# JussiM01/MARL-nav

Hardware: AMD Instinct MI355X
Metric: env-steps/sec (whole node) at 3 agents; 1/2/4/8-GPU scaling + %HBM roofline (higher is better)
Workload: dtype f32

## Files before the change

### marl-nav_amd/csrc/device_math.h

```cpp
#pragma once

__host__ __device__ inline int obs_dim(int A, int O) { return 2 + 2 * O + 2 * (A - 1); }

__device__ __forceinline__ float clamp_t(float x, float lo, float hi)
{
    x = x < lo ? lo : x;
    return x > hi ? hi : x;
}

constexpr bool kNtRows = true;
constexpr bool kNtOther = false;
typedef float v4f_t __attribute__((ext_vector_type(4)));
typedef float v2f_t __attribute__((ext_vector_type(2)));

template <class T>
__device__ __forceinline__ __attribute__((address_space(1))) T *gptr(T *p)
{
    return (__attribute__((address_space(1))) T *)p;
}

template <bool NT = kNtOther, class T>
__device__ __forceinline__ void out_st(T *p, T v)
{
    if constexpr (NT)
// ... 661 lines not shown
#pragma unroll
                for (int l = 0; l < 8; ++l) acc[k][l] += f(x[(4 * r + k) * 8 + l]);
#pragma unroll
        for (int v = 4 * M; v < V; ++v)
#pragma unroll
            for (int l = 0; l < 8; ++l) acc[0][l] += f(x[v * 8 + l]);
#pragma unroll
        for (int k = 1; k < 4; ++k)
#pragma unroll
            for (int l = 0; l < 8; ++l) acc[0][l] += acc[k][l];
        float fin = 0.0f;
#pragma unroll
        for (int i = 8 * V; i < N; ++i) fin += f(x[i]);
#pragma unroll
        for (int l = 0; l < 8; ++l) fin += acc[0][l];
        return fin;
    } else {
        float a0 = 0.0f, a1 = 0.0f, a2 = 0.0f, a3 = 0.0f;
        constexpr int M = N / 4;
#pragma unroll
        for (int r = 0; r < M; ++r) {
            a0 += f(x[4 * r]);
            a1 += f(x[4 * r + 1]);
            a2 += f(x[4 * r + 2]);
            a3 += f(x[4 * r + 3]);
        }
#pragma unroll
        for (int i = 4 * M; i < N; ++i) a0 += f(x[i]);
        a0 += a1;
        a0 += a2;
        a0 += a3;
        return a0;
    }
}

template <bool FAST, bool REFC = false>
__device__ __forceinline__ float bond_term(float d, const MarlnavParams &pr, bool &ok)
{
    if constexpr (FAST) {
        if constexpr (REFC) {
            const float sd = d - pr.ideal_dist;
            return recip_fast(1.0f + sd * sd, ok);
        } else {
            const DivC d_sharp = make_divc(pr.bond_sharpness, ok);
            const float sd = div_c(d - pr.ideal_dist, d_sharp, ok);
            return recip_fast(1.0f + sd * sd, ok);
        }
    } else {
        const float sd = (d - pr.ideal_dist) / pr.bond_sharpness;
        return 1.0f / (1.0f + sd * sd);
    }
}

template <int A, bool FAST, bool REFC>
__device__ __forceinline__ RowOut row_reward(float ta, float td, bool risk_any, bool col_any,
                                             float band, float bond, const MarlnavParams &pr,
                                             bool &ok)
{
    const float head = fabsf(ta) < pr.max_angle_diff ? 1.0f : 0.0f;
    const float bandc = band < pr.max_at_prop_d ? band : pr.max_at_prop_d;
    float dsc, soft;
    if (FAST && (pr.flags & kTermsFastFlag)) {
        const DivC d_init = make_divc(pr.init_dist, ok);
        soft = -1.0f * div_c(td, d_init, ok);
        if constexpr (REFC) {
            dsc = bandc * 0.5f;
        } else {
            const DivC d_mapd = make_divc(pr.max_at_prop_d, ok);
            dsc = div_c(bandc, d_mapd, ok);
        }
    } else {
        dsc = bandc / pr.max_at_prop_d;
        soft = -1.0f * (td / pr.init_dist);
    }
    const float bondm = bond / (float)(A - 1);
    const float risk = risk_any ? 1.0f : 0.0f;
    float rm = pr.target_factor * 0.0f + pr.heading_factor * head;
    float rh = pr.target_factor * 1.0f + pr.heading_factor * head;
    rm = rm + pr.distance_factor * dsc;
    rh = rh + pr.distance_factor * dsc;
    rm = rm + pr.soft_factor * soft;
    rh = rh + pr.soft_factor * soft;
    rm = rm + pr.bond_factor * bondm;
    rh = rh + pr.bond_factor * bondm;
    rm = rm - pr.risk_factor * risk;
    rh = rh - pr.risk_factor * risk;
    return RowOut{rm, rh, (col_any ? 1u : 0u) | ((td < pr.target_radius) ? 2u : 0u)};
}

template <int A, int O, bool TERMS, bool FAST, bool REFC = false>
__device__ __forceinline__ RowOut observe_row_own(const float *__restrict__ sts,
                                                  const float *__restrict__ obe,
                                                  const float *__restrict__ tge, int a,
                                                  float ox, float oy, float dx, float dy,
                                                  float *row, const MarlnavParams &pr, bool &ok)
{
    const float cap = pr.cap_distance;
    if constexpr (FAST) {
        constexpr int NP = 1 + O + (A - 1);
        float px[NP], py[NP], pd[NP], pg[NP];
        px[0] = tge[0];
        py[0] = tge[1];
#pragma unroll
        for (int j = 0; j < O; ++j) {
            px[1 + j] = obe[2 * j];
            py[1 + j] = obe[2 * j + 1];
        }
#pragma unroll
        for (int j = 0; j < A - 1; ++j) {
            const int m = j + (j >= a ? 1 : 0);
            px[1 + O + j] = sts[5 * m];
            py[1 + O + j] = sts[5 * m + 1];
        }
        pairs_fast<NP>(ox, oy, dx, dy, px, py, cap, pd, pg);
        row[0] = pg[0];
        row[1] = pd[0];
        bool ob_risk = false, ob_col = false, ag_risk = false, ag_col = false;
        float band = 0.0f;
#pragma unroll
        for (int j = 0; j < O; ++j) {
            row[2 + j] = pg[1 + j];
            row[2 + O + j] = pd[1 + j];
            if (TERMS) {
                ob_risk |= pd[1 + j] < pr.ob_risk_dist;
                ob_col |= pd[1 + j] < pr.ob_coll_dist;
            }
        }
#pragma unroll
        for (int j = 0; j < A - 1; ++j) {
            const float d = pd[1 + O + j];
            row[2 + 2 * O + j] = pg[1 + O + j];
            row[2 + 2 * O + (A - 1) + j] = d;
            if (TERMS) {
                ag_risk |= d < pr.ag_risk_dist;
                ag_col |= d < pr.ag_coll_dist;
                band += (pr.agents_min_d < d && d < pr.agents_max_d) ? 1.0f : 0.0f;
            }
        }
        RowOut out{0.0f, 0.0f, 0u};
        if (TERMS) {
            const float *agd = row + 2 + 2 * O + (A - 1);
            float bond;
            if (pr.flags & kTermsFastFlag)
                bond = torch_row_sum_r<A - 1>(agd, [&](float d) { return bond_term<true, REFC>(d, pr, ok); });
            else
                bond = torch_row_sum_r<A - 1>(agd, [&](float d) { return bond_term<false>(d, pr, ok); });
            out = row_reward<A, FAST, REFC>(pg[0], pd[0], ob_risk || ag_risk, ob_col || ag_col, band,
                                            bond, pr, ok);
        }
        return out;
    }
    const float td = pair_dist<false>(ox, oy, tge[0], tge[1], ok);
    const float ta = pair_angle<false>(ox, oy, tge[0], tge[1], dx, dy, td, cap, ok);
    row[0] = ta;
    row[1] = td;
    bool ob_risk = false, ob_col = false;
#pragma unroll
    for (int j = 0; j < O; ++j) {
        const float px = obe[2 * j], py = obe[2 * j + 1];
        const float d = pair_dist<false>(ox, oy, px, py, ok);
        row[2 + j] = pair_angle<false>(ox, oy, px, py, dx, dy, d, cap, ok);
        row[2 + O + j] = d;
        if (TERMS) {
            ob_risk |= d < pr.ob_risk_dist;
            ob_col |= d < pr.ob_coll_dist;
        }
    }
    bool ag_risk = false, ag_col = false;
    float band = 0.0f;
#pragma unroll
    for (int j = 0; j < A - 1; ++j) {
        const int m = j + (j >= a ? 1 : 0);
        const float px = sts[5 * m], py = sts[5 * m + 1];
        const float d = pair_dist<false>(ox, oy, px, py, ok);
        row[2 + 2 * O + j] = pair_angle<false>(ox, oy, px, py, dx, dy, d, cap, ok);
        row[2 + 2 * O + (A - 1) + j] = d;
        if (TERMS) {
            ag_risk |= d < pr.ag_risk_dist;
            ag_col |= d < pr.ag_coll_dist;
            band += (pr.agents_min_d < d && d < pr.agents_max_d) ? 1.0f : 0.0f;
        }
    }
    RowOut out{0.0f, 0.0f, 0u};
    if (TERMS) {
        const float *agd = row + 2 + 2 * O + (A - 1);
        const float bond = torch_row_sum_r<A - 1>(agd, [&](float d) { return bond_term<false>(d, pr, ok); });
        out = row_reward<A, false, REFC>(ta, td, ob_risk || ag_risk, ob_col || ag_col, band, bond,
                                         pr, ok);
    }
    return out;
}

template <int A, int O, bool TERMS, bool FAST>
__device__ __forceinline__ RowOut observe_row_regs(const float *__restrict__ sts,
                                                   const float *__restrict__ obe,
                                                   const float *__restrict__ tge, int a,
                                                   float *row, const MarlnavParams &pr,
                                                   bool &ok)
{
    return observe_row_own<A, O, TERMS, FAST>(sts, obe, tge, a, sts[5 * a], sts[5 * a + 1],
                                              sts[5 * a + 2], sts[5 * a + 3], row, pr, ok);
// ... 81 lines not shown
```

### marl-nav_amd/csrc/kernel_args.h

```cpp
#pragma once

typedef __attribute__((address_space(3))) void LdsVoid;

struct KArgs {
    StepArgs a;
    MarlnavParams p;
};
typedef __attribute__((address_space(4))) const KArgs KArgsK;

template <int OFF>
__device__ __forceinline__ KArgsK *kargs_late()
{
    const char *p = (const char *)__builtin_amdgcn_kernarg_segment_ptr() + OFF;
    KArgsK *k = (KArgsK *)p;
    asm volatile("" : "+s"(k));
    return k;
}

constexpr int kHotKargsOff = 7 * 8;

template <class T>
__device__ __forceinline__ T in_sgpr(T p)
{
    asm volatile("" : "+s"(p));
// ... 23 lines not shown
    q.formation = K->a.b.formation;
    return q;
}

__device__ __forceinline__ MarlnavParams load_params(KArgsK *K)
{
    MarlnavParams p;
#define MARLNAV_CP(f) p.f = K->p.f
    MARLNAV_CP(min_speed); MARLNAV_CP(max_speed); MARLNAV_CP(min_accel); MARLNAV_CP(max_accel);
    MARLNAV_CP(trunc_after); MARLNAV_CP(risk_factor); MARLNAV_CP(distance_factor);
    MARLNAV_CP(heading_factor); MARLNAV_CP(target_factor); MARLNAV_CP(soft_factor);
    MARLNAV_CP(bond_factor); MARLNAV_CP(ob_risk_dist); MARLNAV_CP(ag_risk_dist);
    MARLNAV_CP(ob_coll_dist); MARLNAV_CP(ag_coll_dist); MARLNAV_CP(agents_min_d);
    MARLNAV_CP(agents_max_d); MARLNAV_CP(max_at_prop_d); MARLNAV_CP(max_angle_diff);
    MARLNAV_CP(target_radius); MARLNAV_CP(cap_distance); MARLNAV_CP(bond_sharpness);
    MARLNAV_CP(ideal_dist); MARLNAV_CP(init_dist); MARLNAV_CP(obs_range_x);
    MARLNAV_CP(obs_mean_x); MARLNAV_CP(obs_range_y); MARLNAV_CP(obs_mean_y);
    MARLNAV_CP(ags_dist); MARLNAV_CP(noise_std); MARLNAV_CP(angle_range);
    MARLNAV_CP(flags); MARLNAV_CP(seed);
    MARLNAV_CP(act_scale[0]); MARLNAV_CP(act_scale[1]);
    MARLNAV_CP(act_mean[0]); MARLNAV_CP(act_mean[1]);
#undef MARLNAV_CP
    p.reserved = 0;
    return p;
}

template <int NB, int AUX = 0>
__device__ __forceinline__ void glds_span(const void *src, float *dst, unsigned lane)
{
    constexpr int N16 = NB / 16, R4 = (NB % 16) / 4;
#pragma unroll
    for (int k = 0; k * 64 < N16; ++k) {
        const char *s = in_sgpr(reinterpret_cast<const char *>(src) + k * 1024);
        if ((k + 1) * 64 <= N16 || (int)lane < N16 - k * 64)
            __builtin_amdgcn_global_load_lds(s + lane * 16u, (LdsVoid *)(dst + k * 256), 16, 0,
                                             AUX);
    }
    if constexpr (R4 > 0) {
        const char *s = in_sgpr(reinterpret_cast<const char *>(src) + N16 * 16);
        if ((int)lane < R4)
            __builtin_amdgcn_global_load_lds(s + lane * 4u, (LdsVoid *)(dst + N16 * 4), 4, 0,
                                             AUX);
    }
}

typedef float f32x2 __attribute__((ext_vector_type(2)));
__device__ __forceinline__ f32x2 global_load_x2_raw(const float *p)
{
    f32x2 v;
    asm volatile("global_load_dwordx2 %0, %1, off" : "=v"(v) : "v"(p) : "memory");
    return v;
}

__device__ __forceinline__ f32x2 vm_landed(f32x2 v)
{
    asm volatile("" : "+v"(v)::"memory");
    return v;
}

__device__ __forceinline__ void wait_vmcnt(int n)
{
    switch (n) {
    case 0: asm volatile("s_waitcnt vmcnt(0)" ::: "memory"); break;
    case 1: asm volatile("s_waitcnt vmcnt(1)" ::: "memory"); break;
    case 2: asm volatile("s_waitcnt vmcnt(2)" ::: "memory"); break;
    case 3: asm volatile("s_waitcnt vmcnt(3)" ::: "memory"); break;
    case 4: asm volatile("s_waitcnt vmcnt(4)" ::: "memory"); break;
    case 5: asm volatile("s_waitcnt vmcnt(5)" ::: "memory"); break;
    case 6: asm volatile("s_waitcnt vmcnt(6)" ::: "memory"); break;
    case 7: asm volatile("s_waitcnt vmcnt(7)" ::: "memory"); break;
    default: asm volatile("s_waitcnt vmcnt(0)" ::: "memory"); break;
    }
}

template <class T>
__device__ __forceinline__ void copy_span(const T *__restrict__ src, T *__restrict__ dst, int n,
                                          int lane)
{
#pragma clang loop vectorize(disable) unroll(disable)
    for (int i = lane; i < n; i += 64) dst[i] = src[i];
}

__host__ __device__ constexpr int tile_envs(int A) { return (64 / A) >= 4 ? (64 / A) & ~3 : 64 / A; }
```

### marl-nav_amd/csrc/kernel_block.h

```cpp
#pragma once

template <int A, int O>
struct BlockPlan {
    static constexpr int E = 64, R = E * A, D = 2 + 2 * O + 2 * (A - 1);
    static constexpr int NT = 64 * A;
    static constexpr int ST = 0;
    static constexpr int ACTW = (ST + R * 5 + 3) & ~3;
    static constexpr int OB = (ACTW + 2 * R + 3) & ~3;
    static constexpr int TG = (OB + E * O * 2 + 3) & ~3;
    static constexpr int SN = (TG + E * 2 + 3) & ~3;
    static constexpr int TM = (SN + E + 3) & ~3;
    static constexpr int FORM = (TM + E / 4 + 3) & ~3;
    static constexpr int RED = (FORM + 5 * A + 2 + 3) & ~3;
    static constexpr int OBS = RED + 4 * R;
    static constexpr int LIST = (OBS + R * D + 3) & ~3;
    static constexpr int FLG = LIST + E;
    static constexpr int FRESH = (FLG + 1 + A + 3) & ~3;
    static constexpr int FLOATS = FRESH + 2 * O * E;
    static_assert(A >= 2 && A <= 16, "one wave per agent");
};

template <int NB, int AUX = 0>
__device__ __forceinline__ void block_glds(int k, int A, int w, const void *src, float *dst,
                                           unsigned lane)
{
    if (k % A == w) glds_span<NB, AUX>(src, dst, lane);
}

__host__ __device__ constexpr int glds_count(int NB)
{
    return (NB / 16 + 63) / 64 + ((NB % 16) / 4 > 0 ? 1 : 0);
}

template <int A, int O>
struct BlockSpans {
    using BP = BlockPlan<A, O>;
    static constexpr int N = 6;
    static constexpr int K[N] = {0, 1, 4, 2, 5, 7};
    static constexpr int NB[N] = {BP::R * 20, BP::E * O * 8, BP::E * 8, BP::E * 4, BP::E,
                                  (5 * A + 2) * 4};
    static constexpr int after_actions(int w, bool formation)
    {
        int n = 0;
        for (int i = 0; i < N; ++i)
            if (K[i] % A == w && (i != N - 1 || formation)) n += glds_count(NB[i]);
        return n;
    }
};

template <int A, int O, bool OBS_ONLY, int W>
__device__ __forceinline__ void block_stage_wave(const StepPtrs &b, int64_t e0, float *lds,
                                                 unsigned lane, bool formation)
{
    using BP = BlockPlan<A, O>;
    using BS = BlockSpans<A, O>;
    if constexpr (BS::K[0] % A == W)
        glds_span<BS::NB[0]>(b.states + e0 * (A * 5), lds + BP::ST, lane);
    if constexpr (BS::K[1] % A == W)
        glds_span<BS::NB[1]>(b.obstacles + e0 * (O * 2), lds + BP::OB, lane);
    if constexpr (BS::K[2] % A == W) glds_span<BS::NB[2]>(b.target + e0 * 2, lds + BP::TG, lane);
    if constexpr (!OBS_ONLY) {
        if constexpr (BS::K[3] % A == W) glds_span<BS::NB[3]>(b.step_num + e0, lds + BP::SN, lane);
        if constexpr (BS::K[4] % A == W) glds_span<BS::NB[4]>(b.terminates + e0, lds + BP::TM, lane);
        if constexpr (BS::K[5] % A == W)
            if (formation) glds_span<BS::NB[5]>(b.formation, lds + BP::FORM, lane);
    }
}

template <int A, int O, bool OBS_ONLY, int... W>
__device__ __forceinline__ void block_stage_waves(std::integer_sequence<int, W...>, int w,
                                                  const StepPtrs &b, int64_t e0, float *lds,
                                                  unsigned lane, bool formation)
{
    ((w == W ? block_stage_wave<A, O, OBS_ONLY, W>(b, e0, lds, lane, formation) : (void)0), ...);
}

template <int A, int O>
constexpr bool kBlockWaveStage = O < 8;

template <class T>
__device__ __forceinline__ void block_copy(const T *__restrict__ src, T *__restrict__ dst, int n,
                                           int tid, int nt)
{
#pragma clang loop vectorize(disable) unroll(disable)
    for (int i = tid; i < n; i += nt) dst[i] = src[i];
}

__device__ __forceinline__ void block_store(float *__restrict__ dst, const float *__restrict__ src,
                                            int n, int tid, int nt, bool wt)
{
    const int n4 = n >> 2;
    if (wt) {
        const OutBuf ob = out_buf(dst, (uint32_t)n * 4u);
        for (int i = tid; i < n4; i += nt)
            wt_st4(ob, 16u * i, reinterpret_cast<const float4 *>(src)[i]);
        for (int i = (n4 << 2) + tid; i < n; i += nt) wt_st(ob, 4u * i, src[i]);
        return;
    }
    for (int i = tid; i < n4; i += nt)
        out_st4<kNtRows>(dst + 4 * i, reinterpret_cast<const float4 *>(src)[i]);
    for (int i = (n4 << 2) + tid; i < n; i += nt) out_st<kNtRows>(dst + i, src[i]);
}

template <int N1, int N2, int NT>
__device__ __forceinline__ void block_store2(float *__restrict__ d1, const float *__restrict__ s1,
                                             float *__restrict__ d2, const float *__restrict__ s2,
                                             int tid, bool wt)
{
    static_assert(N1 % 4 == 0 && N2 % 4 == 0, "whole 16-byte pieces");
    constexpr int Q1 = N1 / 4, Q2 = N2 / 4, K1 = (Q1 + NT - 1) / NT, K2 = (Q2 + NT - 1) / NT;
    float4 v1[K1], v2[K2];
#pragma unroll
    for (int k = 0; k < K1; ++k)
        if ((k + 1) * NT <= Q1 || tid + k * NT < Q1)
            v1[k] = reinterpret_cast<const float4 *>(s1)[tid + k * NT];
#pragma unroll
    for (int k = 0; k < K2; ++k)
        if ((k + 1) * NT <= Q2 || tid + k * NT < Q2)
            v2[k] = reinterpret_cast<const float4 *>(s2)[tid + k * NT];
    if (wt) {
        const OutBuf o1 = out_buf(d1, N1 * 4), o2 = out_buf(d2, N2 * 4);
#pragma unroll
        for (int k = 0; k < K1; ++k)
            if ((k + 1) * NT <= Q1 || tid + k * NT < Q1) wt_st4(o1, 16u * (tid + k * NT), v1[k]);
#pragma unroll
        for (int k = 0; k < K2; ++k)
            if ((k + 1) * NT <= Q2 || tid + k * NT < Q2) wt_st4(o2, 16u * (tid + k * NT), v2[k]);
        return;
    }
#pragma unroll
    for (int k = 0; k < K1; ++k)
        if ((k + 1) * NT <= Q1 || tid + k * NT < Q1) out_st4<kNtRows>(d1 + 4 * (tid + k * NT), v1[k]);
#pragma unroll
    for (int k = 0; k < K2; ++k)
        if ((k + 1) * NT <= Q2 || tid + k * NT < Q2) out_st4<kNtRows>(d2 + 4 * (tid + k * NT), v2[k]);
}

struct EnvEnd {
    unsigned any_col, all_in;
    float step_num;
    bool truncated, term_old, terminated, fin;
};

template <int A, class F>
__device__ __forceinline__ EnvEnd env_end(F flag, float step_num_old, uint8_t terminates_old,
                                          float trunc_after)
{
    EnvEnd e;
    e.any_col = 0u;
    e.all_in = 1u;
#pragma unroll
    for (int i = 0; i < A; ++i) {
        const unsigned f = flag(i);
        e.any_col |= f & 1u;
        e.all_in &= (f >> 1) & 1u;
    }
    e.step_num = step_num_old + 1.0f;
    e.truncated = e.step_num > trunc_after;
    e.term_old = terminates_old != 0;
    e.terminated = e.any_col != 0u || e.term_old;
    e.fin = e.truncated || e.terminated;
    return e;
}

template <int A, int O, bool HELP>
constexpr bool kBlockEarlyOut = O >= 8 || !HELP;

struct BlockDynamic {
    static constexpr int all_full = -1, write_through = -1, native_overlap = -1,
                         has_formation = -1, no_norm = -1, no_action_scale = -1,
                         default_bond = -1, has_counters = -1;
    static constexpr bool ptrs_early = false;
};

template <bool WT>
struct BlockFixed {
    static constexpr int all_full = 1, write_through = WT, native_overlap = 1, has_formation = 1,
                         no_norm = 1, no_action_scale = 1, default_bond = 1, has_counters = 1;
    static constexpr bool ptrs_early = true;
};


template <int A, int O, bool OBS_ONLY, bool NOISY, bool HELP = false, class FX = BlockDynamic>
__global__ void __launch_bounds__(64 * (A + HELP))
    block_kernel(float *h_states, const float *h_actions, const float *h_obstacles,
                 const float *h_target, const float *h_step_num, const uint8_t *h_terminates,
                 int64_t h_P, KArgs k)
{
    using BP = BlockPlan<A, O>;
    constexpr int E = BP::E, R = BP::R, D = BP::D, NT = BP::NT;
    static_assert(!HELP || (!OBS_ONLY && !NOISY), "the draw wave serves the native re-init step");
    static_assert(FX::native_overlap <= 0 || (!OBS_ONLY && !NOISY), "native_overlap: the native step");
    (void)k;
    extern __shared__ __attribute__((aligned(16))) float lds[];
#if MARLNAV_STAMPS
    unsigned long long t_entry;
    asm volatile("s_memrealtime %0\n\ts_waitcnt lgkmcnt(0)" : "=s"(t_entry));
#endif
    if (MARLNAV_AB & 4096) return;
    const int tid = (int)threadIdx.x;
    const unsigned lane = threadIdx.x & 63;
    const int w = __builtin_amdgcn_readfirstlane(threadIdx.x >> 6);
    const bool hw = HELP && w == A;
    KArgsK *K = kargs_late<kHotKargsOff>();
    const int64_t P = h_P;
    StepPtrs b = load_ptrs(K);
    b.states = h_states;
    b.actions = h_actions;
    b.obstacles = const_cast<float *>(h_obstacles);
    b.target = const_cast<float *>(h_target);
    b.step_num = const_cast<float *>(h_step_num);
    b.terminates = const_cast<uint8_t *>(h_terminates);
    using BS = BlockSpans<A, O>;
    auto block = [&]() __attribute__((always_inline)) {
    const int64_t blk = blockIdx.x;
    const int64_t gw = blk * (A + HELP) + w;
    STAMP(0);
    STAMP_ISSUED_DECL;
    float *st = lds + BP::ST;
    const int64_t e0 = blk * E;
    const int ne = FX::all_full > 0 ? E : (int)((P - e0) < E ? (P - e0) : E);
    const bool full = FX::all_full < 0 ? ne == E : FX::all_full > 0;
    const auto has_form = [&] {
        return FX::has_formation < 0 ? b.formation != nullptr : FX::has_formation > 0;
    };

    constexpr bool WS = kBlockWaveStage<A, O>;
    float *actw = lds + BP::ACTW + 2 * E * (hw ? 0 : w);
    f32x2 act_own = {0.0f, 0.0f};
    if (!OBS_ONLY && full && !hw) {
        const float *pa = h_actions + ((e0 + lane) * A + w) * 2;
        if constexpr (WS) {
            act_own = global_load_x2_raw(pa);
        } else {
            __builtin_amdgcn_global_load_lds(pa, (LdsVoid *)actw, 4, 0, 0);
            __builtin_amdgcn_global_load_lds(pa + 1, (LdsVoid *)(actw + E), 4, 0, 0);
        }
    }
    static_assert(BS::NB[0] == R * 20 && BS::NB[1] == E * O * 8 && BS::NB[2] == E * 8 &&
                      BS::NB[3] == E * 4 && BS::NB[4] == E && BS::NB[5] == (5 * A + 2) * 4,
                  "span table and LDS plan agree");
    if (WS && full) {
        block_stage_waves<A, O, OBS_ONLY>(std::make_integer_sequence<int, A>{}, w, b, e0, lds, lane,
                                          has_form());
    } else if (full) {
        block_glds<BS::NB[0]>(BS::K[0], A, w, b.states + e0 * (A * 5), st, lane);
        block_glds<BS::NB[1]>(BS::K[1], A, w, b.obstacles + e0 * (O * 2), lds + BP::OB, lane);
        block_glds<BS::NB[2]>(BS::K[2], A, w, b.target + e0 * 2, lds + BP::TG, lane);
        if (!OBS_ONLY) {
            block_glds<BS::NB[3]>(BS::K[3], A, w, b.step_num + e0, lds + BP::SN, lane);
            block_glds<BS::NB[4]>(BS::K[4], A, w, b.terminates + e0, lds + BP::TM, lane);
            if (has_form())
                block_glds<BS::NB[5]>(BS::K[5], A, w, b.formation, lds + BP::FORM, lane);
        }
    } else if (!hw) {
        const int nr = ne * A;
        block_copy(b.states + e0 * (A * 5), st, nr * 5, tid, NT);
        if (!OBS_ONLY && (int)lane < ne) {
            const float *pa = h_actions + ((e0 + lane) * A + w) * 2;
            actw[lane] = pa[0];
            actw[E + lane] = pa[1];
        }
        block_copy(b.obstacles + e0 * (O * 2), lds + BP::OB, ne * O * 2, tid, NT);
        block_copy(b.target + e0 * 2, lds + BP::TG, ne * 2, tid, NT);
        if (!OBS_ONLY) {
            block_copy(b.step_num + e0, lds + BP::SN, ne, tid, NT);
            block_copy(b.terminates + e0, reinterpret_cast<uint8_t *>(lds + BP::TM), ne, tid, NT);
            if (has_form()) block_copy(b.formation, lds + BP::FORM, 5 * A + 2, tid, NT);
        }
    }
    STAMP_ISSUED();
    const MarlnavParams pr = load_params(K);
    const bool wt =
        FX::write_through < 0 ? (pr.flags & kWriteThroughFlag) != 0 : FX::write_through > 0;
    const bool overlap = FX::native_overlap < 0 ? !OBS_ONLY && !NOISY && !K->a.b.fresh_states
                                                : FX::native_overlap > 0;
    constexpr bool kPre = E * O <= NT;
    if constexpr (HELP) {
        if (hw && overlap && (int)lane < ne) {
            KArgsK *kl = kargs_late<kHotKargsOff>();
            const uint64_t sidx = kl->a.step_idx, g = (uint64_t)(kl->a.env_offset + e0) + lane;
            float *pre = lds + BP::FRESH;
            float v[O][2];
#pragma unroll
            for (int j = 0; j < O; ++j)
                native_obst_draw(pr.seed, sidx, g, j, pr.obs_range_x, pr.obs_mean_x, pr.obs_range_y,
                                 pr.obs_mean_y, v[j]);
#pragma unroll
            for (int j = 0; j < O; ++j) {
                pre[(2 * j) * E + lane] = v[j][0];
                pre[(2 * j + 1) * E + lane] = v[j][1];
            }
        }
    } else if (kPre && overlap) {
        KArgsK *kl = kargs_late<kHotKargsOff>();
        const uint64_t sidx = kl->a.step_idx, g0 = (uint64_t)(kl->a.env_offset + e0);
        float *pre = lds + BP::FRESH;
#pragma unroll
        for (int k2 = 0; k2 * NT < E * O; ++k2) {
            const int i = tid + k2 * NT;
            const int l = i % E, j = __builtin_amdgcn_readfirstlane(i / E);
            if (((k2 + 1) * NT <= E * O || i < E * O) && l < ne) {
                float v[2];
                native_obst_draw(pr.seed, sidx, g0 + l, j, pr.obs_range_x, pr.obs_mean_x,
                                 pr.obs_range_y, pr.obs_mean_y, v);
                pre[(2 * j) * E + l] = v[0];
                pre[(2 * j + 1) * E + l] = v[1];
            }
        }
    }
    float sn = 0.0f, c = 1.0f, a1 = 0.0f;
    if (!OBS_ONLY && !hw) {
        if (full) {
            int n = 0;
#pragma unroll
            for (int ww = 0; ww < A; ++ww)
                if (w == ww) n = has_form() ? BS::after_actions(ww, true) : BS::after_actions(ww, false);
            wait_vmcnt(n);
        }
        float a0;
        if (WS && full) {
            act_own = vm_landed(act_own);
            a0 = act_own.x;
            a1 = act_own.y;
        } else {
            a0 = actw[lane];
            a1 = actw[E + lane];
        }
        STAMPS_S(0);
        if (FX::no_action_scale < 0 ? (pr.flags & MARLNAV_SCALE_ACTIONS) != 0
                                    : FX::no_action_scale == 0) {
            KArgsK *kl = kargs_late<kHotKargsOff>();
            a0 = kl->p.act_scale[0] * a0 + kl->p.act_mean[0];
            a1 = kl->p.act_scale[1] * a1 + kl->p.act_mean[1];
        }
        sincos_k(clamp_t(a0, -kPiF, kPiF), &sn, &c);
#if MARLNAV_STAMPS && MARLNAV_SUBSTAMPS
        asm volatile("" ::"v"(sn), "v"(c));
#endif
        STAMPS_S(1);
    }
    const int l = (int)lane;
    const int r = l * A + (hw ? 0 : w);
    const bool row_on = l < ne && !hw;
    const int nrow = ne * A;
    int *bad_word = reinterpret_cast<int *>(lds + BP::FLG) + 1;
    if (tid == 0) *bad_word = 0;
    asm volatile("s_waitcnt vmcnt(0)" ::: "memory");
    STAMPS_S(2);
    __syncthreads();
    STAMP(1);
    if (MARLNAV_AB & 8192) {
        asm volatile("" ::"v"(sn), "v"(c), "v"(a1));
        return;
    }

    CoordRange crange;
    if (full && !hw) {
        constexpr int NC = E * O * 2 + E * 2;
        static_assert(BP::TG == BP::OB + E * O * 2, "adjacent obstacle/target spans");
#pragma unroll
        for (int k2 = 0; k2 * NT < NC; ++k2) {
            const int i = tid + k2 * NT;
            if ((k2 + 1) * NT <= NC || i < NC) crange.add(lds[BP::OB + i]);
        }
    }

    float ox, oy, dx, dy;
    {
        const float *s = st + 5 * r;
        ox = s[0];
        oy = s[1];
        dx = s[2];
        dy = s[3];
    }
    if (!OBS_ONLY) {
        const float ndx = c * dx + (-sn) * dy;
        const float ndy = sn * dx + c * dy;
        float *s = st + 5 * r;
        const float v = clamp_t(s[4] + clamp_t(a1, pr.min_accel, pr.max_accel), pr.min_speed,
                                pr.max_speed);
        ox = ox + ndx * v;
        oy = oy + ndy * v;
        dx = ndx;
        dy = ndy;
        if (row_on) {
            s[0] = ox;
            s[1] = oy;
            s[2] = dx;
            s[3] = dy;
            s[4] = v;
        }
    }
    if (full && !hw) {
        crange.add(ox);
        crange.add(oy);
        const bool bad = __ballot(!crange.ok()) != 0ull;
        if (lane == 0 && bad) *bad_word = 1;
    }
    __syncthreads();
    STAMP(2);
    const bool fast = full && *bad_word == 0;

    float4 *red = reinterpret_cast<float4 *>(lds + BP::RED);
    float *obs_rows = lds + BP::OBS;
    if (row_on) {
        float rowv[D];
        RowOut ro;
        bool unused = true;
        if (__builtin_expect(fast, 1) &&
            (FX::default_bond < 0 ? pr.bond_sharpness == 1.0f && pr.max_at_prop_d == 2.0f
                                  : FX::default_bond > 0))
            ro = observe_row_own<A, O, !OBS_ONLY, true, true>(st + 5 * A * l, lds + BP::OB + 2 * O * l,
                                                              lds + BP::TG + 2 * l, w, ox, oy, dx,
                                                              dy, rowv, pr, unused);
        else if (FX::default_bond <= 0 && __builtin_expect(fast, 1))
            ro = observe_row_own<A, O, !OBS_ONLY, true>(st + 5 * A * l, lds + BP::OB + 2 * O * l,
                                                        lds + BP::TG + 2 * l, w, ox, oy, dx, dy,
                                                        rowv, pr, unused);
        else
            ro = observe_row_own<A, O, !OBS_ONLY, false>(st + 5 * A * l, lds + BP::OB + 2 * O * l,
                                                         lds + BP::TG + 2 * l, w, ox, oy, dx, dy,
                                                         rowv, pr, unused);
#if MARLNAV_STAMPS && MARLNAV_SUBSTAMPS
        asm volatile("" ::"v"(ro.r_miss), "v"(rowv[0]), "v"(rowv[D - 1]));
#endif
        STAMPS_S(3);
        lds_row_write<D>(obs_rows + r * D, rowv);
        if (!OBS_ONLY) red[r] = make_float4(ro.r_miss, ro.r_hit, __uint_as_float(ro.flags), 0.0f);
    }
    StepPtrs bo;
    uint64_t *cnt_early = nullptr;
    int64_t slots_early = 0;
    if constexpr (FX::ptrs_early) {
        KArgsK *kl = kargs_late<kHotKargsOff>();
        bo = load_ptrs(kl);
        cnt_early = in_sgpr(kl->a.b.counters);
        slots_early = in_sgpr(kl->a.waves);
    }
    __syncthreads();
    STAMP(3);
    if (MARLNAV_AB & 16384) return;
    if constexpr (!FX::ptrs_early) bo = load_ptrs(kargs_late<kHotKargsOff>());
    float *gobs = in_sgpr(bo.obs + e0 * (A * D));
    if (OBS_ONLY) block_store(gobs, obs_rows, nrow * D, tid, NT, wt);
    const bool norm = !OBS_ONLY && (FX::no_norm < 0 ? (pr.flags & MARLNAV_WRITE_OBS_NORM) != 0
                                                    : FX::no_norm == 0);
    bool early = false;
    if (!OBS_ONLY) {
        int *list = reinterpret_cast<int *>(lds + BP::LIST);
        int *flg = reinterpret_cast<int *>(lds + BP::FLG);
        const BlockEnvs<A, O, D> ev{st, lds + BP::OB, lds + BP::TG, obs_rows, e0};
        if (w == 0) {
            __builtin_amdgcn_s_setprio(3);
            const bool env_on = l < ne;
            bool fin = false, tr_l = false, co_l = false, ta_l = false;
            if (env_on) {
                const int64_t e = e0 + l;
                float rx[A], ry[A];
                unsigned rf[A];
#pragma unroll
                for (int i = 0; i < A; ++i) {
                    const float4 t = red[A * l + i];
                    rx[i] = t.x;
                    ry[i] = t.y;
                    rf[i] = __float_as_uint(t.z);
                }
                const EnvEnd ee = env_end<A>([&](int i) { return rf[i]; }, lds[BP::SN + l],
                                             reinterpret_cast<const uint8_t *>(lds + BP::TM)[l],
                                             pr.trunc_after);
                const unsigned any_col = ee.any_col, all_in = ee.all_in;
                float rv[A];
// ... 193 lines not shown
```

### marl-nav_amd/csrc/marlnav_debug.h

```cpp
#pragma once

#ifndef MARLNAV_STAMPS
#define MARLNAV_STAMPS 0
#endif
#if MARLNAV_STAMPS
__device__ unsigned long long *g_stamps;
typedef __attribute__((address_space(1))) unsigned long long stamp_t;
#define STAMP_PTR(off) ((stamp_t *)(g_stamps) + (off))
#define STAMP(k)                                                                   \
    do {                                                                           \
        if (lane == 0) {                                                           \
            stamp_t *sp_ = STAMP_PTR((size_t)gw * 24);                             \
            sp_[2 * (k)] = wall_clock64();                                         \
            sp_[2 * (k) + 1] = clock64();                                          \
        }                                                                          \
    } while (0)
#ifndef MARLNAV_SUBSTAMPS
#define MARLNAV_SUBSTAMPS 0
#endif
#define STAMP_SLOT_(k)                                                             \
    do {                                                                           \
        if (lane == 0) *STAMP_PTR((size_t)gw * 24 + 20 + (k)) = wall_clock64();    \
    } while (0)
#if MARLNAV_SUBSTAMPS
#define STAMPX(k) \
    do {          \
    } while (0)
#if MARLNAV_SUBSTAMPS == 2
#define STAMPS_S(k)                       \
    do {                                  \
        if ((k) != 3) STAMP_SLOT_(k);     \
    } while (0)
#define STAMP_ISSUED_DECL unsigned long long t_issued = 0
#define STAMP_ISSUED() \
    asm volatile("s_memrealtime %0\n\ts_waitcnt lgkmcnt(0)" : "=s"(t_issued)::"memory")
#define STAMP_ISSUED_STORE()                                           \
    do {                                                               \
        if (lane == 0) *STAMP_PTR((size_t)gw * 24 + 23) = t_issued;    \
    } while (0)
#else
#define STAMPS_S(k) STAMP_SLOT_(k)
#endif
#else
#define STAMPX(k) STAMP_SLOT_(k)
#define STAMPS_S(k) \
    do {            \
    } while (0)
#endif
#else
#define STAMPS_S(k) \
    do {            \
    } while (0)
#define STAMPX(k) \
    do {          \
    } while (0)
#define STAMP(k) \
    do {         \
    } while (0)
#endif
#ifndef STAMP_ISSUED
#define STAMP_ISSUED_DECL \
    do {                  \
    } while (0)
#define STAMP_ISSUED() \
    do {               \
    } while (0)
#define STAMP_ISSUED_STORE() \
    do {                     \
    } while (0)
#endif

#ifndef MARLNAV_AB
#define MARLNAV_AB 0
#endif
```

### marl-nav_amd/csrc/marlnav_step.hip

```cpp
#include <hip/hip_runtime.h>

#include <atomic>
#include <type_traits>
#include <utility>

#include <stdarg.h>
#include <stdint.h>
#include <stdio.h>
#include <stdlib.h>
#include <string.h>

#include "../../include/marlnav.h"

namespace {

constexpr float kPiF = 3.14159265358979323846f;
constexpr int kMaxAgents = 64;
constexpr int kMaxStride = 256;
constexpr int kWavesPerBlock = 4;
constexpr int kWaveLdsFloats = 4096;
constexpr int kObsTileMax = 2304;

#include "marlnav_debug.h"

// ... 279 lines not shown
    if (n <= 0) {
        if (hipDeviceGetAttribute(&n, hipDeviceAttributeMultiprocessorCount, dev) != hipSuccess ||
            n <= 0)
            n = 256;
        cached[dev].store(n, std::memory_order_relaxed);
    }
    return n;
}

template <int A, int O>
constexpr BlockFn block_draw_fn()
{
    if constexpr (O <= 3) return block_kernel<A, O, false, false, true>;
    else return nullptr;
}

template <int A, int O, bool WT>
constexpr BlockFn block_fixed_draw_fn()
{
    if constexpr (O <= 3) return block_kernel<A, O, false, false, true, BlockFixed<WT>>;
    else return nullptr;
}

#define MARLNAV_BLOCK_VARIANT(A, O)                                                    \
    {A, O, block_kernel<A, O, false, false>, block_kernel<A, O, true, false>,          \
     block_kernel<A, O, false, true>, (size_t)BlockPlan<A, O>::FLOATS * 4,             \
     block_draw_fn<A, O>(), BlockPlan<A, O>::E, {nullptr, nullptr}, {nullptr, nullptr}}
#define MARLNAV_BLOCK_VARIANT_FIXED(A, O)                                              \
    {A, O, block_kernel<A, O, false, false>, block_kernel<A, O, true, false>,          \
     block_kernel<A, O, false, true>, (size_t)BlockPlan<A, O>::FLOATS * 4,             \
     block_draw_fn<A, O>(), BlockPlan<A, O>::E,                                        \
     {block_kernel<A, O, false, false, false, BlockFixed<false>>,                      \
      block_kernel<A, O, false, false, false, BlockFixed<true>>},                      \
     {block_fixed_draw_fn<A, O, false>(), block_fixed_draw_fn<A, O, true>()}}
const BlockVariant kBlockVariants[] = {
    MARLNAV_BLOCK_VARIANT_FIXED(3, 3),
    MARLNAV_BLOCK_VARIANT_FIXED(3, 8),
    MARLNAV_BLOCK_VARIANT(3, 1),
    MARLNAV_BLOCK_VARIANT(2, 1),
};
#undef MARLNAV_BLOCK_VARIANT
#undef MARLNAV_BLOCK_VARIANT_FIXED

const BlockVariant *select_block(const MarlnavDims *d, const MarlnavStepBuffers &b, bool obs_only)
{
    if (d->obstacle_stride != d->num_obstacles) return nullptr;
    const BlockVariant *v = nullptr;
    for (const BlockVariant &x : kBlockVariants)
        if (x.A == d->num_agents && x.O == d->num_obstacles) v = &x;
    if (!v) return nullptr;
    if (!aligned(b.states, 16) || !aligned(b.obstacles, 16) || !aligned(b.target, 16) ||
        !aligned(b.obs, 16) || (b.states_out && !aligned(b.states_out, 16)))
        return nullptr;
    if (!obs_only && (!aligned(b.actions, 16) || !aligned(b.step_num, 16) ||
                      !aligned(b.terminates, 16) || (b.formation && !aligned(b.formation, 16))))
        return nullptr;
    return v;
}

int launch_block(const BlockVariant &v, BlockFn fn, const StepArgs &args, const MarlnavParams &pr,
                 void *stream, const char *what, int waves = 0)
{
    KArgs ka;
    ka.a = args;
    ka.p = pr;
    ka.a.W = v.E;
    ka.a.ntiles = (args.P + ka.a.W - 1) / ka.a.W;
    float *h_states = args.b.states;
    const float *h_actions = args.b.actions, *h_obstacles = args.b.obstacles,
                *h_target = args.b.target, *h_step_num = args.b.step_num;
    const uint8_t *h_terminates = args.b.terminates;
    int64_t h_P = args.P;
    void *kargs[] = {&h_states, &h_actions, &h_obstacles, &h_target, &h_step_num, &h_terminates,
                     &h_P, &ka};
    hipError_t e = hipLaunchKernel(reinterpret_cast<const void *>(fn), dim3((unsigned)ka.a.ntiles),
                                   dim3(64 * (waves ? waves : v.A)), kargs, v.lds, (hipStream_t)stream);
    if (e == hipSuccess) e = hipGetLastError();
    if (e != hipSuccess) return fail(MARLNAV_ELAUNCH, "%s: %s", what, hipGetErrorString(e));
    return 0;
}

bool has_variant(int A, int O)
{
    for (const KernelPair &k : kVariants)
        if (k.A == A && k.O == O) return true;
    return false;
}

KernelPair select_kernels(int A, int O)
{
    for (const KernelPair &k : kVariants)
        if (k.A == A && k.O == O) return k;
    return KernelPair{0, 0, wave_kernel<0, 0, false>, wave_kernel<0, 0, true>,
                      wave_kernel<0, 0, false, true>};
}

StepArgs make_args(const MarlnavDims *d, const Launch &L)
{
    StepArgs a;
    memset(&a, 0, sizeof(a));
    a.P = d->num_parallel;
    a.env_offset = d->env_offset;
    a.ntiles = L.ntiles;
    a.waves = L.waves;
    a.W = L.W;
    a.A = d->num_agents;
    a.O = d->num_obstacles;
    a.S = d->obstacle_stride;
    return a;
}

int launch(StepFn fn, const Launch &L, StepArgs args, MarlnavParams pr, void *stream,
           const char *what)
{
    void *kargs[] = {&args, &pr};
    const size_t lds = (size_t)L.plan.floats * 4 * kWavesPerBlock;
    hipError_t e = hipLaunchKernel(reinterpret_cast<const void *>(fn), dim3((unsigned)L.blocks),
                                   dim3(64 * kWavesPerBlock), kargs, lds, (hipStream_t)stream);
    if (e == hipSuccess) e = hipGetLastError();
    if (e != hipSuccess) return fail(MARLNAV_ELAUNCH, "%s: %s", what, hipGetErrorString(e));
    return 0;
}

std::atomic<int> g_family{MARLNAV_FAMILY_AUTO};
thread_local int g_last_family = MARLNAV_FAMILY_AUTO;

bool family_allowed(int f)
{
    const int g = g_family.load(std::memory_order_relaxed);
    return g == MARLNAV_FAMILY_AUTO || g == f;
}

std::atomic<int> g_block_traits{MARLNAV_BLOCK_TRAITS_AUTO};
thread_local int g_last_block_traits = MARLNAV_BLOCK_RAN_GENERAL;

bool block_fixed_eligible(const MarlnavDims *d, const MarlnavParams &pr,
                          const MarlnavStepBuffers &b, const BlockVariant &v, const Launch &L,
                          bool noisy)
{
    const int64_t nblk = (d->num_parallel + v.E - 1) / v.E;
    return d->num_parallel % v.E == 0 && !noisy && !b.fresh_states && b.formation &&
           !(pr.flags & (MARLNAV_WRITE_OBS_NORM | MARLNAV_SCALE_ACTIONS)) &&
           pr.bond_sharpness == 1.0f && pr.max_at_prop_d == 2.0f && b.counters &&
           nblk <= L.waves;
}

}

extern "C" {

int marlnav_abi_version(void) { return MARLNAV_ABI_VERSION; }

int marlnav_debug_force_family(int family)
{
    const int prev = g_family.load(std::memory_order_relaxed);
    if (family < MARLNAV_FAMILY_AUTO || family > MARLNAV_FAMILY_WAVE)
        return fail(MARLNAV_EINVAL, "unknown kernel family %d", family);
    g_family.store(family, std::memory_order_relaxed);
    return prev;
}

int marlnav_debug_last_family(void) { return g_last_family; }

int marlnav_debug_force_block_traits(int mode)
{
    const int prev = g_block_traits.load(std::memory_order_relaxed);
    if (mode < MARLNAV_BLOCK_TRAITS_AUTO || mode > MARLNAV_BLOCK_TRAITS_FIXED_NO_DRAW)
        return fail(MARLNAV_EINVAL, "unknown block traits mode %d", mode);
    g_block_traits.store(mode, std::memory_order_relaxed);
    return prev;
}

int marlnav_debug_last_block_traits(void) { return g_last_block_traits; }

#if MARLNAV_STAMPS
int marlnav_debug_stamps(void *buf)
{
    const hipError_t e = hipMemcpyToSymbol(HIP_SYMBOL(g_stamps), &buf, sizeof(buf));
    return e == hipSuccess ? 0 : fail(MARLNAV_ELAUNCH, "stamps: %s", hipGetErrorString(e));
}
#endif

int marlnav_debug_acos_range(uint32_t first, int64_t n, float *out, void *stream)
{
    if (n < 0 || (n > 0 && !out)) return fail(MARLNAV_EINVAL, "acos range: n < 0 or out NULL");
    if (n == 0) return 0;
    hipLaunchKernelGGL(acos_range_kernel, dim3((unsigned)((n + 255) / 256)), dim3(256), 0,
                       (hipStream_t)stream, first, n, out);
    const hipError_t e = hipGetLastError();
    return e == hipSuccess ? 0 : fail(MARLNAV_ELAUNCH, "acos range: %s", hipGetErrorString(e));
}

int marlnav_debug_fastdiv_check(uint32_t d_first, uint32_t d_stride, uint32_t nd, uint64_t *out,
                                void *stream)
{
    if (nd > 0 && !out) return fail(MARLNAV_EINVAL, "fastdiv check: out NULL");
    if (nd == 0) return 0;
// ... 186 lines not shown
```

Before: 11.51 billion.

## Trim block-kernel prologue with SGPR-based loads, exec-masked LDS staging, static waits

Adds a compile-time prologue bitmask (on by default) for the fixed block variant. It loads actions through an SGPR base plus a lane offset, and issues partial global-to-LDS pieces with exec masks instead of lane branches. It also replaces the dynamic vmcnt counting with per-wave static waits, computes the obstacle-draw indices directly from the lane and wave, and specialises the terms-fast flag at compile time. The aim is to cut scalar and vector instruction overhead and branching in the kernel prologue. In exchange it adds inline asm that depends on exact vmcnt ordering, and it tightens fixed-variant eligibility to require the fast-terms flag.

```diff
diff --git a/marl-nav_amd/csrc/device_math.h b/marl-nav_amd/csrc/device_math.h
--- a/marl-nav_amd/csrc/device_math.h
+++ b/marl-nav_amd/csrc/device_math.h
@@ -737,7 +737,7 @@
     }
 }
 
-template <int A, bool FAST, bool REFC>
+template <int A, bool FAST, bool REFC, int TF = -1>
 __device__ __forceinline__ RowOut row_reward(float ta, float td, bool risk_any, bool col_any,
                                              float band, float bond, const MarlnavParams &pr,
                                              bool &ok)
@@ -745,7 +745,7 @@
     const float head = fabsf(ta) < pr.max_angle_diff ? 1.0f : 0.0f;
     const float bandc = band < pr.max_at_prop_d ? band : pr.max_at_prop_d;
     float dsc, soft;
-    if (FAST && (pr.flags & kTermsFastFlag)) {
+    if (FAST && (TF < 0 ? (pr.flags & kTermsFastFlag) != 0 : TF > 0)) {
         const DivC d_init = make_divc(pr.init_dist, ok);
         soft = -1.0f * div_c(td, d_init, ok);
         if constexpr (REFC) {
@@ -773,7 +773,7 @@
     return RowOut{rm, rh, (col_any ? 1u : 0u) | ((td < pr.target_radius) ? 2u : 0u)};
 }
 
-template <int A, int O, bool TERMS, bool FAST, bool REFC = false>
+template <int A, int O, bool TERMS, bool FAST, bool REFC = false, int TF = -1>
 __device__ __forceinline__ RowOut observe_row_own(const float *__restrict__ sts,
                                                   const float *__restrict__ obe,
                                                   const float *__restrict__ tge, int a,
@@ -826,12 +826,12 @@
         if (TERMS) {
             const float *agd = row + 2 + 2 * O + (A - 1);
             float bond;
-            if (pr.flags & kTermsFastFlag)
+            if (TF < 0 ? (pr.flags & kTermsFastFlag) != 0 : TF > 0)
                 bond = torch_row_sum_r<A - 1>(agd, [&](float d) { return bond_term<true, REFC>(d, pr, ok); });
             else
                 bond = torch_row_sum_r<A - 1>(agd, [&](float d) { return bond_term<false>(d, pr, ok); });
-            out = row_reward<A, FAST, REFC>(pg[0], pd[0], ob_risk || ag_risk, ob_col || ag_col, band,
-                                            bond, pr, ok);
+            out = row_reward<A, FAST, REFC, TF>(pg[0], pd[0], ob_risk || ag_risk, ob_col || ag_col,
+                                                band, bond, pr, ok);
         }
         return out;
     }
diff --git a/marl-nav_amd/csrc/kernel_args.h b/marl-nav_amd/csrc/kernel_args.h
--- a/marl-nav_amd/csrc/kernel_args.h
+++ b/marl-nav_amd/csrc/kernel_args.h
@@ -99,6 +99,13 @@
     return v;
 }
 
+__device__ __forceinline__ f32x2 global_load_x2_raw(const float *base, uint32_t off)
+{
+    f32x2 v;
+    asm volatile("global_load_dwordx2 %0, %1, %2" : "=v"(v) : "v"(off), "s"(base) : "memory");
+    return v;
+}
+
 __device__ __forceinline__ f32x2 vm_landed(f32x2 v)
 {
     asm volatile("" : "+v"(v)::"memory");
@@ -120,6 +127,13 @@
     }
 }
 
+template <int N>
+__device__ __forceinline__ void wait_vmcnt()
+{
+    static_assert(N >= 0 && N < 64, "vmcnt is six bits");
+    asm volatile("s_waitcnt vmcnt(%0)" ::"n"(N) : "memory");
+}
+
 template <class T>
 __device__ __forceinline__ void copy_span(const T *__restrict__ src, T *__restrict__ dst, int n,
                                           int lane)
diff --git a/marl-nav_amd/csrc/kernel_block.h b/marl-nav_amd/csrc/kernel_block.h
--- a/marl-nav_amd/csrc/kernel_block.h
+++ b/marl-nav_amd/csrc/kernel_block.h
@@ -20,8 +20,66 @@
     static_assert(A >= 2 && A <= 16, "one wave per agent");
 };
 
-template <int NB, int AUX = 0>
-__device__ __forceinline__ void block_glds(int k, int A, int w, const void *src, float *dst,
+typedef __attribute__((address_space(3))) float LdsF;
+template <bool MASK>
+struct LdsDst {
+    LdsF *p;
+    __device__ __forceinline__ LdsDst operator+(int n) const { return LdsDst{p + n}; }
+};
+
+template <int N, int B>
+__device__ __forceinline__ void glds_lanes(const char *s, LdsF *d, unsigned voff)
+{
+    static_assert(N > 0 && N < 64 && (B == 4 || B == 16), "a partial piece");
+    const uint32_t m0 = (uint32_t)(uintptr_t)d;
+    if constexpr (B == 16)
+        asm volatile("s_bfm_b64 exec, %2, 0\n\tglobal_load_lds_dwordx4 %0, %1\n\t"
+                     "s_mov_b64 exec, -1" ::"v"(voff), "s"(s), "n"(N), "{m0}"(m0)
+                     : "memory");
+    else
+        asm volatile("s_bfm_b64 exec, %2, 0\n\tglobal_load_lds_dword %0, %1\n\t"
+                     "s_mov_b64 exec, -1" ::"v"(voff), "s"(s), "n"(N), "{m0}"(m0)
+                     : "memory");
+}
+
+template <int NB, int AUX, bool MASK, int K>
+__device__ __forceinline__ void glds_piece(const void *src, LdsDst<MASK> dst, unsigned lane)
+{
+    constexpr int N16 = NB / 16;
+    const char *s = in_sgpr(reinterpret_cast<const char *>(src) + K * 1024);
+    if constexpr ((K + 1) * 64 <= N16)
+        __builtin_amdgcn_global_load_lds(s + lane * 16u, (LdsVoid *)(dst.p + K * 256), 16, 0, AUX);
+    else if constexpr (MASK)
+        glds_lanes<N16 - K * 64, 16>(s, dst.p + K * 256, lane * 16u);
+    else if ((int)lane < N16 - K * 64)
+        __builtin_amdgcn_global_load_lds(s + lane * 16u, (LdsVoid *)(dst.p + K * 256), 16, 0, AUX);
+}
+
+template <int NB, int AUX, bool MASK, int... K>
+__device__ __forceinline__ void glds_pieces(std::integer_sequence<int, K...>, const void *src,
+                                            LdsDst<MASK> dst, unsigned lane)
+{
+    (glds_piece<NB, AUX, MASK, K>(src, dst, lane), ...);
+}
+
+template <int NB, int AUX = 0, bool MASK>
+__device__ __forceinline__ void glds_span(const void *src, LdsDst<MASK> dst, unsigned lane)
+{
+    constexpr int N16 = NB / 16, R4 = (NB % 16) / 4;
+    static_assert(!MASK || AUX == 0, "the masked pieces carry no cache policy");
+    glds_pieces<NB, AUX>(std::make_integer_sequence<int, (N16 + 63) / 64>{}, src, dst, lane);
+    if constexpr (R4 > 0) {
+        const char *s = in_sgpr(reinterpret_cast<const char *>(src) + N16 * 16);
+        if constexpr (MASK)
+            glds_lanes<R4, 4>(s, dst.p + N16 * 4, lane * 4u);
+        else if ((int)lane < R4)
+            __builtin_amdgcn_global_load_lds(s + lane * 4u, (LdsVoid *)(dst.p + N16 * 4), 4, 0,
+                                             AUX);
+    }
+}
+
+template <int NB, int AUX = 0, class DST>
+__device__ __forceinline__ void block_glds(int k, int A, int w, const void *src, DST dst,
                                            unsigned lane)
 {
     if (k % A == w) glds_span<NB, AUX>(src, dst, lane);
@@ -48,8 +106,8 @@
     }
 };
 
-template <int A, int O, bool OBS_ONLY, int W>
-__device__ __forceinline__ void block_stage_wave(const StepPtrs &b, int64_t e0, float *lds,
+template <int A, int O, bool OBS_ONLY, int W, class DST>
+__device__ __forceinline__ void block_stage_wave(const StepPtrs &b, int64_t e0, DST lds,
                                                  unsigned lane, bool formation)
 {
     using BP = BlockPlan<A, O>;
@@ -67,9 +125,9 @@
     }
 }
 
-template <int A, int O, bool OBS_ONLY, int... W>
+template <int A, int O, bool OBS_ONLY, class DST, int... W>
 __device__ __forceinline__ void block_stage_waves(std::integer_sequence<int, W...>, int w,
-                                                  const StepPtrs &b, int64_t e0, float *lds,
+                                                  const StepPtrs &b, int64_t e0, DST lds,
                                                   unsigned lane, bool formation)
 {
     ((w == W ? block_stage_wave<A, O, OBS_ONLY, W>(b, e0, lds, lane, formation) : (void)0), ...);
@@ -169,16 +227,51 @@
 struct BlockDynamic {
     static constexpr int all_full = -1, write_through = -1, native_overlap = -1,
                          has_formation = -1, no_norm = -1, no_action_scale = -1,
-                         default_bond = -1, has_counters = -1;
+                         default_bond = -1, has_counters = -1, terms_fast = -1;
     static constexpr bool ptrs_early = false;
+    static constexpr int prologue = 0;
+};
+
+enum : int {
+    kProActBase = 1,
+    kProLdsPtr = 2,
+    kProExecMask = 4,
+    kProWait = 8,
+    kProDrawW = 16,
+    kProTerms = 32,
 };
 
 template <bool WT>
 struct BlockFixed {
+    static constexpr int prologue = MARLNAV_PROLOGUE;
     static constexpr int all_full = 1, write_through = WT, native_overlap = 1, has_formation = 1,
-                         no_norm = 1, no_action_scale = 1, default_bond = 1, has_counters = 1;
+                         no_norm = 1, no_action_scale = 1, default_bond = 1, has_counters = 1,
+                         terms_fast = (prologue & kProTerms) ? 1 : -1;
     static constexpr bool ptrs_early = true;
 };
+
+template <int PRO>
+__device__ __forceinline__ auto block_lds_dst(float *lds)
+{
+    if constexpr (PRO & (kProLdsPtr | kProExecMask))
+        return LdsDst<(PRO & kProExecMask) != 0>{(LdsF *)lds};
+    else
+        return lds;
+}
+
+template <int A, int O, int W = 0>
+__device__ __forceinline__ void block_wait_actions(int w)
+{
+    constexpr int n = BlockSpans<A, O>::after_actions(W, true);
+    if constexpr (W == A - 1) {
+        wait_vmcnt<n>();
+    } else {
+        if (w == W)
+            wait_vmcnt<n>();
+        else
+            block_wait_actions<A, O, W + 1>(w);
+    }
+}
 
 
 template <int A, int O, bool OBS_ONLY, bool NOISY, bool HELP = false, class FX = BlockDynamic>
@@ -230,7 +323,10 @@
     f32x2 act_own = {0.0f, 0.0f};
     if (!OBS_ONLY && full && !hw) {
         const float *pa = h_actions + ((e0 + lane) * A + w) * 2;
-        if constexpr (WS) {
+        if constexpr (WS && (FX::prologue & kProActBase) != 0) {
+            act_own = global_load_x2_raw(in_sgpr(h_actions + e0 * (2 * A) + 2 * w),
+                                         lane * (8u * A));
+        } else if constexpr (WS) {
             act_own = global_load_x2_raw(pa);
         } else {
             __builtin_amdgcn_global_load_lds(pa, (LdsVoid *)actw, 4, 0, 0);
@@ -240,18 +336,19 @@
     static_assert(BS::NB[0] == R * 20 && BS::NB[1] == E * O * 8 && BS::NB[2] == E * 8 &&
                       BS::NB[3] == E * 4 && BS::NB[4] == E && BS::NB[5] == (5 * A + 2) * 4,
                   "span table and LDS plan agree");
+    const auto ldst = block_lds_dst<FX::prologue>(lds);
     if (WS && full) {
-        block_stage_waves<A, O, OBS_ONLY>(std::make_integer_sequence<int, A>{}, w, b, e0, lds, lane,
+        block_stage_waves<A, O, OBS_ONLY>(std::make_integer_sequence<int, A>{}, w, b, e0, ldst, lane,
                                           has_form());
     } else if (full) {
-        block_glds<BS::NB[0]>(BS::K[0], A, w, b.states + e0 * (A * 5), st, lane);
-        block_glds<BS::NB[1]>(BS::K[1], A, w, b.obstacles + e0 * (O * 2), lds + BP::OB, lane);
-        block_glds<BS::NB[2]>(BS::K[2], A, w, b.target + e0 * 2, lds + BP::TG, lane);
+        block_glds<BS::NB[0]>(BS::K[0], A, w, b.states + e0 * (A * 5), ldst + BP::ST, lane);
+        block_glds<BS::NB[1]>(BS::K[1], A, w, b.obstacles + e0 * (O * 2), ldst + BP::OB, lane);
+        block_glds<BS::NB[2]>(BS::K[2], A, w, b.target + e0 * 2, ldst + BP::TG, lane);
         if (!OBS_ONLY) {
-            block_glds<BS::NB[3]>(BS::K[3], A, w, b.step_num + e0, lds + BP::SN, lane);
-            block_glds<BS::NB[4]>(BS::K[4], A, w, b.terminates + e0, lds + BP::TM, lane);
+            block_glds<BS::NB[3]>(BS::K[3], A, w, b.step_num + e0, ldst + BP::SN, lane);
+            block_glds<BS::NB[4]>(BS::K[4], A, w, b.terminates + e0, ldst + BP::TM, lane);
             if (has_form())
-                block_glds<BS::NB[5]>(BS::K[5], A, w, b.formation, lds + BP::FORM, lane);
+                block_glds<BS::NB[5]>(BS::K[5], A, w, b.formation, ldst + BP::FORM, lane);
         }
     } else if (!hw) {
         const int nr = ne * A;
@@ -299,7 +396,9 @@
 #pragma unroll
         for (int k2 = 0; k2 * NT < E * O; ++k2) {
             const int i = tid + k2 * NT;
-            const int l = i % E, j = __builtin_amdgcn_readfirstlane(i / E);
+            constexpr bool kW = (FX::prologue & kProDrawW) != 0 && E == 64 && NT == 64 * A;
+            const int l = kW ? (int)lane : i % E;
+            const int j = kW ? w + k2 * A : __builtin_amdgcn_readfirstlane(i / E);
             if (((k2 + 1) * NT <= E * O || i < E * O) && l < ne) {
                 float v[2];
                 native_obst_draw(pr.seed, sidx, g0 + l, j, pr.obs_range_x, pr.obs_mean_x,
@@ -311,7 +410,10 @@
     }
     float sn = 0.0f, c = 1.0f, a1 = 0.0f;
     if (!OBS_ONLY && !hw) {
-        if (full) {
+        if constexpr (WS && (FX::prologue & kProWait) != 0 && FX::all_full > 0 &&
+                      FX::has_formation > 0) {
+            block_wait_actions<A, O>(w);
+        } else if (full) {
             int n = 0;
 #pragma unroll
             for (int ww = 0; ww < A; ++ww)
@@ -411,13 +513,13 @@
         if (__builtin_expect(fast, 1) &&
             (FX::default_bond < 0 ? pr.bond_sharpness == 1.0f && pr.max_at_prop_d == 2.0f
                                   : FX::default_bond > 0))
-            ro = observe_row_own<A, O, !OBS_ONLY, true, true>(st + 5 * A * l, lds + BP::OB + 2 * O * l,
-                                                              lds + BP::TG + 2 * l, w, ox, oy, dx,
-                                                              dy, rowv, pr, unused);
+            ro = observe_row_own<A, O, !OBS_ONLY, true, true, FX::terms_fast>(
+                st + 5 * A * l, lds + BP::OB + 2 * O * l, lds + BP::TG + 2 * l, w, ox, oy, dx, dy,
+                rowv, pr, unused);
         else if (FX::default_bond <= 0 && __builtin_expect(fast, 1))
-            ro = observe_row_own<A, O, !OBS_ONLY, true>(st + 5 * A * l, lds + BP::OB + 2 * O * l,
-                                                        lds + BP::TG + 2 * l, w, ox, oy, dx, dy,
-                                                        rowv, pr, unused);
+            ro = observe_row_own<A, O, !OBS_ONLY, true, false, FX::terms_fast>(
+                st + 5 * A * l, lds + BP::OB + 2 * O * l, lds + BP::TG + 2 * l, w, ox, oy, dx, dy,
+                rowv, pr, unused);
         else
             ro = observe_row_own<A, O, !OBS_ONLY, false>(st + 5 * A * l, lds + BP::OB + 2 * O * l,
                                                          lds + BP::TG + 2 * l, w, ox, oy, dx, dy,
diff --git a/marl-nav_amd/csrc/marlnav_debug.h b/marl-nav_amd/csrc/marlnav_debug.h
--- a/marl-nav_amd/csrc/marlnav_debug.h
+++ b/marl-nav_amd/csrc/marlnav_debug.h
@@ -73,3 +73,7 @@
 #ifndef MARLNAV_AB
 #define MARLNAV_AB 0
 #endif
+
+#ifndef MARLNAV_PROLOGUE
+#define MARLNAV_PROLOGUE 63
+#endif
diff --git a/marl-nav_amd/csrc/marlnav_step.hip b/marl-nav_amd/csrc/marlnav_step.hip
--- a/marl-nav_amd/csrc/marlnav_step.hip
+++ b/marl-nav_amd/csrc/marlnav_step.hip
@@ -355,7 +355,7 @@
     if (!aligned(b.states, 16) || !aligned(b.obstacles, 16) || !aligned(b.target, 16) ||
         !aligned(b.obs, 16) || (b.states_out && !aligned(b.states_out, 16)))
         return nullptr;
-    if (!obs_only && (!aligned(b.actions, 16) || !aligned(b.step_num, 16) ||
+    if (!obs_only && (!aligned(b.actions, 8) || !aligned(b.step_num, 16) ||
                       !aligned(b.terminates, 16) || (b.formation && !aligned(b.formation, 16))))
         return nullptr;
     return v;
@@ -445,7 +445,8 @@
     return d->num_parallel % v.E == 0 && !noisy && !b.fresh_states && b.formation &&
            !(pr.flags & (MARLNAV_WRITE_OBS_NORM | MARLNAV_SCALE_ACTIONS)) &&
            pr.bond_sharpness == 1.0f && pr.max_at_prop_d == 2.0f && b.counters &&
-           nblk <= L.waves;
+           nblk <= L.waves &&
+           (BlockFixed<false>::terms_fast < 0 || (pr.flags & kTermsFastFlag) != 0);
 }
 
 }
```

Result: faster. 11.64 billion, median of 6 (+1.1%).
